# polimi-ispl/deep_prior_interpolation

Hardware: AMD Instinct MI355X
Metric: Adam iters/sec on 3D MultiRes-UNet (whole job over n_gpus; per_gpu beside it); recon SNR(dB) vs ref under config.snr_vs_reference (higher is better)
Workload: dtype f32

## Files before the change

### deep_prior_interpolation_amd/csrc/api.cpp

```cpp
#include <stdarg.h>
#include <string.h>
#include "common.h"

static thread_local char g_err[512] = "";

void dpi_set_error(const char* fmt, ...) {
  va_list ap;
  va_start(ap, fmt);
  vsnprintf(g_err, sizeof(g_err), fmt, ap);
  va_end(ap);
}

int dpi_check_launch(const char* what) {
  const hipError_t e = hipGetLastError();
  if (e != hipSuccess) {
    dpi_set_error("%s: %s", what, hipGetErrorString(e));
    return DPI_E_LAUNCH;
  }
  return DPI_OK;
}

extern "C" const char* dpi_last_error(void) { return g_err; }
extern "C" int dpi_version(void) { return 406; }
extern "C" int dpi_conv_desc_size(void) { return (int)sizeof(dpi_conv_desc); }

extern "C" int dpi_device_info(int device, int* cus, int* lds_bytes, size_t* hbm_bytes, char* name, int name_len) {
  hipDeviceProp_t p;
  const hipError_t e = hipGetDeviceProperties(&p, device);
  if (e != hipSuccess) {
    dpi_set_error("device_info: %s", hipGetErrorString(e));
    return DPI_E_LAUNCH;
  }
  if (cus) *cus = p.multiProcessorCount;
  if (lds_bytes) *lds_bytes = (int)p.sharedMemPerBlock;
  if (hbm_bytes) *hbm_bytes = p.totalGlobalMem;
  if (name && name_len > 0) {
    strncpy(name, p.gcnArchName, name_len - 1);
    name[name_len - 1] = 0;
  }
  return DPI_OK;
}

__global__ void dpi_marker_kernel() {}

extern "C" int dpi_profile_marker(int id, void* stream) {
  DPI_REQUIRE(id >= 1 && id < 65536, "profile_marker: id %d out of range", id);
  dpi_marker_kernel<<<(unsigned)id, 64, 0, (hipStream_t)stream>>>();
  return dpi_check_launch("profile_marker");
}

extern "C" int dpi_set_option(const char* key, int value) {
  DPI_REQUIRE(key != nullptr, "set_option: key is NULL");
  struct Entry { const char* key; int lo, hi; void (*set)(int); };
  static const Entry table[] = {
      {"splitk", 0, 1, dpi_set_splitk},
      {"dual_bwd_data", 0, 1, dpi_set_dual_bwd_data},
      {"bw_pair", 0, 2, dpi_set_bw_pair},
      {"bw_workgroups", 1, 1 << 24, [](int v) { dpi_set_bw_tuning(v, -1); }},
      {"bw_xcd_order", 0, 1, [](int v) { dpi_set_bw_tuning(0, v); }},
      {"mfma_min_cout", 0, 1 << 20, dpi_set_mfma_min_cout},
      {"bwd_weight_mfma_min_cout", 0, 1 << 20, dpi_set_bwd_weight_mfma_min_cout},
      {"fewco_mfma", 0, 1, dpi_set_fewco_mfma},
      {"q4", 0, 2, [](int v) { dpi_set_q4(v, -1); }},
      {"q4_ck", 0, 4, [](int v) { dpi_set_q4(-1, v); }},
      {"q4_debug", 0, 0xFFFF, dpi_set_q4_debug},
      {"bf16_debug", 0, 0x7F, dpi_set_bf16_debug},
  };
  for (const Entry& e : table)
    if (strcmp(key, e.key) == 0) {
      DPI_REQUIRE(value >= e.lo && value <= e.hi && !(strcmp(key, "q4_ck") == 0 && value != 0 && value != 2 && value != 4),
                  "set_option: %s = %d out of range [%d, %d]", key, value, e.lo, e.hi);
      e.set(value);
      return DPI_OK;
    }
  dpi_set_error("set_option: unknown key '%s'", key);
  return DPI_E_ARG;
}
```

### deep_prior_interpolation_amd/csrc/conv_mfma.hip

```cpp
#include "conv_kernels.h"

namespace {

typedef float f32x4 __attribute__((ext_vector_type(4)));

struct MArgs {
  const float* __restrict__ x;
  const float* __restrict__ chain;
  const float* __restrict__ w;
  const float* __restrict__ bias;
  float* __restrict__ y;
  double* __restrict__ partials;
  int Cin, Cout;
  int D, H, W;
  int ntd, nth, ntw;
  long w_out_stride, w_in_stride;
  int accumulate;
  int split_cps;
  const float* __restrict__ x2;
  const float* __restrict__ w2;
  int C2;
  long w2_co_stride, w2_c_stride;
  int xb, yb;
  int ny;
// ... 143 lines not shown
#pragma unroll
      for (int e = 0; e < GV::E; ++e)
        if ((e + 1) * 256 <= GV::NV4 || loff[e] >= 0) {
          float* const p = lds + c * GV::CS + loff[e];
          *reinterpret_cast<f32x2*>(p) = (f32x2){sv[c][e][0], sv[c][e][2]};
          *reinterpret_cast<f32x2*>(p + GV::PW) = (f32x2){sv[c][e][1], sv[c][e][3]};
        }
    return;
  }
#pragma unroll
  for (int c = 0; c < 4; ++c) {
    const Chain t = load_chain(chain, min(c0 + c, Cin - 1));
#pragma unroll
    for (int e = 0; e < GV::E; ++e) {
      const float m = goff[e] >= 0 ? 1.f : 0.f;
      if ((e + 1) * 256 <= GV::NV4 || loff[e] >= 0) {
        float* const p = lds + c * GV::CS + loff[e];
        *reinterpret_cast<f32x2*>(p) = (f32x2){m * apply_chain(t, sv[c][e][0]), m * apply_chain(t, sv[c][e][2])};
        *reinterpret_cast<f32x2*>(p + GV::PW) = (f32x2){m * apply_chain(t, sv[c][e][1]), m * apply_chain(t, sv[c][e][3])};
      }
    }
  }
}

#ifdef DPI_TRACE
__device__ long long g_blk[8192][4];
__device__ long long g_trace[4][64];
#define TR(i) do { if (trc >= 0 && tid == 0) g_trace[trc][i] = clock64(); } while (0)
#define TRC(i) do { if (trc >= 0 && tid == 0 && (i) < 38) g_trace[trc][i] = clock64(); } while (0)
#else
#define TR(i)
#define TRC(i)
#endif
template <int KD, int NR, int NH, bool FLIP, int S = 1, int WPE = 2, bool PERSIST = false, bool TAILPACK = false, bool IOB = false, bool YLOOP = false,
          bool S2V = false>
__global__ __launch_bounds__(256, WPE) void conv_mfma_kernel(MArgs a) {
  static_assert(!YLOOP || (!PERSIST && !TAILPACK), "the channel-tile loop is built for the one-tile-per-workgroup variants without a packed tail");
  static_assert(!S2V || (S == 2 && !FLIP && !PERSIST && !TAILPACK && !IOB && NR < 4), "vectorised stride-2 staging: forward, fp32 tensors, row-split tiles");
  using GV = GeoV2<KD, NR < 4 ? NR : 2, NH>;
  if constexpr (!IOB) { a.xb = 0; a.yb = 0; }
  using G = Geo<KD, NR, NH, S>;
  constexpr int TAPS = KD * 9;
  constexpr int PD = (KD - 1) / 2;
  constexpr int NT = NR * NH;
  __shared__ __attribute__((aligned(16))) float lds[4 * (S2V ? GV::CS : G::CS)];
  __shared__ double red[4][16][2];

  const int tid = threadIdx.x, lane = tid & 63, wid = tid >> 6;
  const int lk = lane >> 4, lj = lane & 15;
  const int ntiles = a.ntd * a.nth * a.ntw;
  int vt0 = blockIdx.x, ytile = blockIdx.y;
  if constexpr (!PERSIST) {
    if (a.ny > 0) {
      const int q8 = ntiles >> 3, r8 = ntiles & 7, xcd = blockIdx.x & 7, j = blockIdx.x >> 3;
      const int i = YLOOP ? j : j / a.ny;
      ytile = YLOOP ? 0 : j - i * a.ny;
      if (i >= q8 + (xcd < r8 ? 1 : 0)) return;
      vt0 = i * 8 + xcd;
    }
  }
  int n0 = ytile * 16;
  const size_t V = (size_t)a.D * a.H * a.W;
  const int Do = (a.D + 2 * PD - KD) / G::SD + 1, Ho = (a.H - 1) / S + 1, Wo = (a.W - 1) / S + 1;
  const size_t Vo = (size_t)Do * Ho * Wo;
#ifdef DPI_TRACE
  const int trc = blockIdx.y != 0 ? -1 : blockIdx.x == 0 ? 0 : blockIdx.x == 1 ? 1 : blockIdx.x == 30 ? 2 : blockIdx.x == 50 ? 3 : -1;
  TR(0);
  if (tid == 0 && blockIdx.y == 0 && blockIdx.x < 8192) {
    g_blk[blockIdx.x][0] = wall_clock64();
    g_blk[blockIdx.x][2] = __builtin_amdgcn_s_getreg(63492);
    g_blk[blockIdx.x][3] = __builtin_amdgcn_s_getreg(63508);
  }
#endif
  auto tile_origin = [&](int vt, int& tile_id, int& od0, int& oh0, int& ow0) {
    tile_id = xcd_tile(vt, ntiles);
    int bt = tile_id;
    const int tw_i = bt % a.ntw; bt /= a.ntw;
    const int th_i = bt % a.nth; bt /= a.nth;
    od0 = bt * G::TZ; oh0 = th_i * G::TY; ow0 = tw_i * G::TW;
  };

  const int wz = G::SLICES ? wid : 0, wh = G::SLICES ? 0 : wid * NR;
  const int lbase = S2V ? lk * GV::CS + wh * 2 * GV::RS + lj : lk * G::CS + wz * G::SD * G::DS + wh * S * G::RS + lj * S;

  int co_w = n0 + lj;
  auto w_ptr = [&](int c0, bool& ok) {
    const int ci = c0 + lk;
    ok = co_w < a.Cout && ci < a.Cin;
    return a.w + (ok ? co_w : 0) * a.w_out_stride + (ok ? ci : 0) * a.w_in_stride;
  };
  auto load_w_raw = [&](float (&wn)[9], int c0, int kd) {
    bool ok;
    const float* __restrict__ wp = w_ptr(c0, ok);
#pragma unroll
    for (int t = 0; t < 9; ++t) wn[t] = wp[FLIP ? (TAPS - 1 - (kd * 9 + t)) : kd * 9 + t];
  };
  auto commit_w = [&](float (&wr)[TAPS], const float (&wn)[9], int c0, int kd) {
    const bool ok = co_w < a.Cout && c0 + lk < a.Cin;
#pragma unroll
    for (int t = 0; t < 9; ++t) wr[kd * 9 + t] = ok ? wn[t] : 0.f;
  };

  const int c_lo = a.split_cps ? (int)blockIdx.z * a.split_cps : 0;
  float* __restrict__ const ybase = a.y + (size_t)blockIdx.z * a.Cout * Vo;
  constexpr int EE = S2V ? GV::E : G::E;
  int goff[EE], loff[EE];
  float wr[TAPS], wn[9], sr[S2V ? 1 : 4][S2V ? 1 : G::E];
  f32x4 sv[S2V ? 4 : 1][S2V ? GV::E : 1];
  auto slots = [&](int od, int oh, int ow) {
    if constexpr (S2V) tile_slots_v<GV>(tid, od * G::SD - PD, oh * 2 - 1, ow * 2 - 4, a.D, a.H, a.W, goff, loff);
    else tile_slots<G>(tid, od * G::SD - PD, oh * S - 1, ow * S - 1, a.D, a.H, a.W, goff, loff);
  };
  auto sload = [&](int c0) {
    if constexpr (S2V) stage_load_v<GV>(sv, a.x, a.Cin, V, c0, goff);
    else stage_load<G>(sr, a.x, a.Cin, V, c0, goff, a.xb);
  };
  auto sstore = [&](int c0) {
    if constexpr (S2V) stage_store_v<GV>(lds, sv, a.chain, a.Cin, c0, goff, loff);
    else stage_store<G>(lds, sr, a.chain, a.Cin, c0, goff, loff, a.xb);
  };
  int vt = vt0, tile_id, od0, oh0, ow0;
  tile_origin(vt, tile_id, od0, oh0, ow0);
  slots(od0, oh0, ow0);
  sload(c_lo);
  {
    bool ok;
    const float* __restrict__ wp = w_ptr(c_lo, ok);
#pragma unroll
    for (int t = 0; t < TAPS; ++t) wr[t] = wp[FLIP ? (TAPS - 1 - t) : t];
#pragma unroll
    for (int t = 0; t < TAPS; ++t) wr[t] = ok ? wr[t] : 0.f;
  }

  constexpr int NTG = (TAPS + 3) / 4;
  const bool tail = TAILPACK && S == 1 && (a.Cin & 3) == 1 && (a.Cin > 4 || a.Cin == 1);
  const int cin_main = a.split_cps ? min(c_lo + a.split_cps, a.Cin) : (tail ? a.Cin - 1 : a.Cin);
  int ttoff[TAILPACK ? NTG : 1];
  float wt[TAILPACK ? NTG : 1];
  if constexpr (TAILPACK) {
#pragma unroll
    for (int g = 0; g < NTG; ++g) {
      const int t = 4 * g + lk;
      const int kd = t / 9, kh = (t / 3) % 3, kw = t % 3;
      ttoff[g] = t < TAPS ? kd * G::DS + kh * G::RS + kw : 0;
      wt[g] = 0.f;
    }
  }
  auto load_tail_w = [&]() {
    if constexpr (TAILPACK) {
      const bool ok = co_w < a.Cout;
      const float* __restrict__ wp = a.w + (ok ? co_w : 0) * a.w_out_stride + (a.Cin - 1) * a.w_in_stride;
#pragma unroll
      for (int g = 0; g < NTG; ++g) {
        const int t = 4 * g + lk < TAPS ? 4 * g + lk : TAPS - 1;
        wt[g] = wp[FLIP ? (TAPS - 1 - t) : t];
      }
    }
  };
  auto commit_tail_w = [&]() {
    if constexpr (TAILPACK) {
#pragma unroll
      for (int g = 0; g < NTG; ++g) wt[g] = (co_w < a.Cout && 4 * g + lk < TAPS) ? wt[g] : 0.f;
    }
  };

  for (;;) {
    const int vt_next = vt + (int)gridDim.x;
    const bool has_next = PERSIST && vt_next < ntiles;
    int tile_n = 0, od_n = 0, oh_n = 0, ow_n = 0;
    if (has_next) tile_origin(vt_next, tile_n, od_n, oh_n, ow_n);

    const int nyt = YLOOP ? a.ny : 1;
    for (int yt = 0; yt < nyt; ++yt) {
    if constexpr (YLOOP) {
      if (yt > 0) {
        n0 = yt * 16; co_w = n0 + lj;
        const bool ok = co_w < a.Cout && c_lo + lk < a.Cin;
#pragma unroll
        for (int t = 0; t < TAPS; ++t) wr[t] = ok ? wr[t] : 0.f;
      }
    }
    f32x4 acc[NT];
#pragma unroll
    for (int t = 0; t < NT; ++t) acc[t] = (f32x4){0.f, 0.f, 0.f, 0.f};
    if (a.accumulate) {
#pragma unroll
      for (int r = 0; r < 4; ++r) {
        const int co = n0 + 4 * lk + r;
#pragma unroll
        for (int t = 0; t < NT; ++t) {
          const int od = od0 + wz, oh = oh0 + wh + t / NH, ow = ow0 + (t % NH) * 16 + lj;
          if (co < a.Cout && od < Do && oh < Ho && ow < Wo) acc[t][r] = dpi_ld(ybase, (size_t)co * Vo + ((size_t)od * Ho + oh) * Wo + ow, a.yb);
        }
      }
    }

    TR(1);
    for (int c0 = c_lo; c0 < cin_main; c0 += 4) {
      if (!YLOOP || yt == 0) {
      __syncthreads();
      TRC(2 + (c0 / 4) * 4);
      sstore(c0);
      TRC(3 + (c0 / 4) * 4);
      __syncthreads();
      TRC(4 + (c0 / 4) * 4);
      }
      const bool more = c0 + 4 < cin_main;
      const bool tail_next = tail && !more;
      if (more || tail_next) sload(c0 + 4);
      else if (has_next) {
        slots(od_n, oh_n, ow_n);
        sload(c_lo);
      }
      float bc[G::NB], bn[G::NB];
      auto load_b = [&](float (&b)[G::NB], int step) {
        const int kd = step / G::NROW, ir = step % G::NROW;
#pragma unroll
        for (int h = 0; h < NH; ++h)
#pragma unroll
          for (int kw = 0; kw < 3; ++kw) {
            if constexpr (S2V)
              b[h * 3 + kw] = lds[lbase + kd * GV::DS + ir * GV::RS + h * 16 + (kw == 1 ? 2 : GV::PW + (kw == 0 ? 1 : 2))];
            else b[h * 3 + kw] = lds[lbase + kd * G::DS + ir * G::RS + h * 16 * S + kw];
          }
      };
      load_b(bc, 0);
      const int cn = more ? c0 + 4 : c_lo;
      if (tail_next) load_tail_w();
#pragma unroll
      for (int step = 0; step < G::NSTEP; ++step) {
        const int kd = step / G::NROW, ir = step % G::NROW;
        if (step + 1 < G::NSTEP) load_b(bn, step + 1);
        if constexpr (!YLOOP) { if (ir == 0) load_w_raw(wn, cn, kd); }
        if (WPE <= 2) __builtin_amdgcn_sched_barrier(0);
#pragma unroll
        for (int kw = 0; kw < 3; ++kw)
#pragma unroll
          for (int kh = 0; kh < 3; ++kh) {
            const int hr = (ir - kh) / S;
            if (ir - kh >= 0 && (ir - kh) % S == 0 && hr < NR) {
#pragma unroll
              for (int h = 0; h < NH; ++h)
                acc[hr * NH + h] = __builtin_amdgcn_mfma_f32_16x16x4f32(wr[(kd * 3 + kh) * 3 + kw], bc[h * 3 + kw], acc[hr * NH + h], 0, 0, 0);
            }
          }
        if (WPE <= 2) __builtin_amdgcn_sched_barrier(0);
#pragma unroll
        for (int i = 0; i < G::NB; ++i) bc[i] = bn[i];
        if constexpr (!YLOOP) { if (ir == G::NROW - 1) commit_w(wr, wn, cn, kd); }
      }
      if (tail_next) commit_tail_w();
      TRC(5 + (c0 / 4) * 4);
    }
    if constexpr (TAILPACK) {
      if (tail && cin_main == 0) { load_tail_w(); commit_tail_w(); }
      if (tail) {
        __syncthreads();
        sstore(cin_main);
        __syncthreads();
        if (has_next) {
          slots(od_n, oh_n, ow_n);
          sload(0);
        }
#pragma unroll
        for (int hr = 0; hr < NR; ++hr) {
          float tb[NH][NTG];
#pragma unroll
          for (int h = 0; h < NH; ++h)
#pragma unroll
            for (int g = 0; g < NTG; ++g) tb[h][g] = lds[lbase + ttoff[g] + hr * G::RS + h * 16];
#pragma unroll
          for (int g = 0; g < NTG; ++g)
#pragma unroll
            for (int h = 0; h < NH; ++h)
              acc[hr * NH + h] = __builtin_amdgcn_mfma_f32_16x16x4f32(wt[g], tb[h][g], acc[hr * NH + h], 0, 0, 0);
        }
      }
    }
    if constexpr (YLOOP) {
      if (yt + 1 < nyt) {
        const int con = (yt + 1) * 16 + lj, ci = c_lo + lk;
        const bool okn = con < a.Cout && ci < a.Cin;
        const float* __restrict__ wp = a.w + (okn ? con : 0) * a.w_out_stride + (okn ? ci : 0) * a.w_in_stride;
#pragma unroll
        for (int t = 0; t < TAPS; ++t) wr[t] = wp[FLIP ? (TAPS - 1 - t) : t];
      }
    }
    if constexpr (FLIP && !PERSIST) if (a.x2 != nullptr) {
      const __amdgpu_buffer_rsrc_t r2 = dpi_buffer_t(a.x2, (size_t)a.C2 * Vo, a.xb);
      int voff[NT];
#pragma unroll
      for (int t = 0; t < NT; ++t) {
        const int od = od0 + wz, oh = oh0 + wh + t / NH, ow = ow0 + (t % NH) * 16 + lj;
        voff[t] = (od < Do && oh < Ho && ow < Wo) ? (od * Ho + oh) * Wo + ow : -1;
      }
      const int nk2 = (a.C2 + 3) >> 2;
      auto load2 = [&](float (&b)[NT], float& wv, int kc) {
        const int c = kc * 4 + lk;
        const bool ok = c < a.C2 && co_w < a.Cout;
        const float wraw = a.w2[(ok ? co_w : 0) * a.w2_co_stride + (ok ? c : 0) * a.w2_c_stride];
        wv = ok ? wraw : 0.f;
        const int cbase = c * (int)Vo;
#pragma unroll
        for (int t = 0; t < NT; ++t)
          b[t] = a.xb ? dpi_buffer_load_bf16(r2, voff[t] >= 0 ? cbase + voff[t] : -1) : dpi_buffer_load(r2, voff[t] >= 0 ? (cbase + voff[t]) * 4 : -4);
      };
      float b0[NT], b1[NT], w0v, w1v;
      load2(b0, w0v, 0);
      for (int kc = 0; kc < nk2; kc += 2) {
        if (kc + 1 < nk2) load2(b1, w1v, kc + 1);
#pragma unroll
        for (int t = 0; t < NT; ++t) acc[t] = __builtin_amdgcn_mfma_f32_16x16x4f32(w0v, b0[t], acc[t], 0, 0, 0);
        if (kc + 1 < nk2) {
          if (kc + 2 < nk2) load2(b0, w0v, kc + 2);
#pragma unroll
          for (int t = 0; t < NT; ++t) acc[t] = __builtin_amdgcn_mfma_f32_16x16x4f32(w1v, b1[t], acc[t], 0, 0, 0);
        }
      }
    }
    TR(40);

    const bool interior = od0 + G::TZ <= Do && oh0 + G::TY <= Ho && ow0 + G::TW <= Wo && n0 + 16 <= a.Cout;
    const int vbase = ((od0 + wz) * Ho + oh0 + wh) * Wo + ow0 + lj;
#pragma unroll
    for (int r = 0; r < 4; ++r) {
      const int co = n0 + 4 * lk + r;
      const bool cok = co < a.Cout;
      const float bv = (a.bias && cok) ? a.bias[co] : 0.f;
      float* __restrict__ yc = dpi_at(ybase, (size_t)(cok ? co : 0) * Vo + vbase, a.yb);
      double s = 0.0, q = 0.0;
      if (a.yb) {
        const bool pairs = !(Wo & 1) && !(Vo & 1) && !((uintptr_t)ybase & 3);
#pragma unroll
        for (int t = 0; t < NT; ++t) {
          const int od = od0 + wz, oh = oh0 + wh + t / NH, ow = ow0 + (t % NH) * 16 + lj;
          const bool ok = interior || (cok && od < Do && oh < Ho && ow < Wo);
          const float v = dpi_round_bf16(acc[t][r] + bv);
          dpi_st_bf16_row(yc, (t / NH) * Wo + (t % NH) * 16, v, ok, pairs, lj);
          if (ok) { s += v; q += (double)v * v; }
        }
      } else if (interior) {
#pragma unroll
        for (int t = 0; t < NT; ++t) {
          const float v = acc[t][r] + bv;
          yc[(t / NH) * Wo + (t % NH) * 16] = v;
          if (a.partials) { s += v; q += (double)v * v; }
        }
      } else {
#pragma unroll
        for (int t = 0; t < NT; ++t) {
          const int od = od0 + wz, oh = oh0 + wh + t / NH, ow = ow0 + (t % NH) * 16 + lj;
          if (cok && od < Do && oh < Ho && ow < Wo) {
            const float v = acc[t][r] + bv;
            yc[(t / NH) * Wo + (t % NH) * 16] = v;
            s += v;
            q += (double)v * v;
          }
        }
      }
      if (a.partials) {
#pragma unroll
        for (int o = 8; o > 0; o >>= 1) { s += __shfl_xor(s, o, 64); q += __shfl_xor(q, o, 64); }
        if (lj == 0) { red[wid][4 * lk + r][0] = s; red[wid][4 * lk + r][1] = q; }
      }
    }
    if (a.partials) {
      __syncthreads();
      if (tid < 32) {
        const int c = tid >> 1, which = tid & 1;
        const double rsum = red[0][c][which] + red[1][c][which] + red[2][c][which] + red[3][c][which];
        if (n0 + c < a.Cout) a.partials[((size_t)tile_id * a.Cout + n0 + c) * 2 + which] = rsum;
      }
    }
    }
    TR(41);
    if (!has_next) break;
    vt = vt_next; tile_id = tile_n; od0 = od_n; oh0 = oh_n; ow0 = ow_n;
  }
#ifdef DPI_TRACE
  if (tid == 0 && blockIdx.y == 0 && blockIdx.x < 8192) g_blk[blockIdx.x][1] = wall_clock64();
#endif
}

struct BwMArgs {
  const float* __restrict__ x;
  const float* __restrict__ chain;
  const float* __restrict__ dy;
  float* __restrict__ ws;
  int Cin, Cout;
  int D, H, W;
  int ntd, nth, ntw, ntiles, tiles_per_chunk;
  int swap;
  int y0;
  int ngroups, nchunks;
  int xb, dyb;
};

template <int KD, int S, int NR, int NH, int NG = 1>
struct BwLds {
  using G = Geo<KD, NR, NH, S>;
  static constexpr int NTQ0 = (4 * KD * 9 + 15) / 16;
  static constexpr int LDSF = NG * (4 * G::CS > 4 * NTQ0 * 256 ? 4 * G::CS : 4 * NTQ0 * 256);
  static constexpr int DYRS = 4 * (4 * NH) + 4;
};

template <int KD, int S, int NR, int NH, int TC, int NG = 1, bool IOB = false>
__device__ __forceinline__ void conv_bwd_weight_mfma_body(const BwMArgs& a_in, float* __restrict__ lds, float* __restrict__ dyl_all, int first_group = -1) {
  BwMArgs a = a_in;
  if constexpr (!IOB) { a.xb = 0; a.dyb = 0; }
  static_assert(NG == 1 || TC == 0, "the column-trimmed tail is a single group");
#ifdef DPI_TRACE
  const int trc = (blockIdx.y == 0 && blockIdx.z == 0 && blockIdx.x < 4) ? (int)blockIdx.x : -1;
  int trn = 0;
#define TRW() do { if (trc >= 0 && threadIdx.x == 0 && trn < 64) g_trace[trc][trn++] = clock64(); } while (0)
// ... 551 lines not shown
  }
}

}

static void dpi_mfma_variant(const dpi_conv_desc* d, int cout, int* nr, int* nh) {
  int Do, Ho, Wo;
  dpi_conv_out_dims(d, &Do, &Ho, &Wo);
  const int tz = d->kd == 3 ? 4 : 1, ty = d->kd == 3 ? 8 : 32;
  const long nb = (long)cdiv(Do, tz) * cdiv(Ho, ty) * cdiv(Wo, 32) * cdiv(cout, 16);
  if (nb >= 512 && d->stride == 1) { *nr = 8; *nh = 2; }
  else { *nr = 2; *nh = Wo > 16 ? 2 : 1; }
}

static bool dpi_mfma_half_tile(const dpi_conv_desc* d, bool flip) {
  const int cin = flip ? d->Cout : d->Cin, cout = flip ? d->Cin : d->Cout;
  int nr, nh;
  dpi_mfma_variant(d, cout, &nr, &nh);
  if (nr != 8 || d->kd != 3) return false;
  if (cin == 1) return true;
  if (cin <= 8) return false;
  return flip || ((cin & 3) == 1);
}

static int dpi_mfma_tiles(const dpi_conv_desc* d, int nr, int nh, int* ntd, int* nth, int* ntw) {
  int Do, Ho, Wo;
  dpi_conv_out_dims(d, &Do, &Ho, &Wo);
  const bool slices = d->kd == 3 && nr >= 4;
  const int tz = slices ? 4 : 1, ty = slices ? nr : 4 * nr;
  *ntd = cdiv(Do, tz); *nth = cdiv(Ho, ty); *ntw = cdiv(Wo, 16 * nh);
  return *ntd * *nth * *ntw;
}

struct MfmaTiling { int nr, nh, ntd, nth, ntw, ntiles; };
static MfmaTiling mfma_tiling(const dpi_conv_desc* d, bool flip) {
  MfmaTiling t{};
  dpi_mfma_variant(d, flip ? d->Cin : d->Cout, &t.nr, &t.nh);
  if (dpi_mfma_half_tile(d, flip)) t.nr = 4;
  t.ntiles = dpi_mfma_tiles(d, t.nr, t.nh, &t.ntd, &t.nth, &t.ntw);
  return t;
}
int dpi_conv_mfma_stat_blocks(const dpi_conv_desc* d, bool flip) { return mfma_tiling(d, flip).ntiles; }

template <int KD, bool FLIP, bool IOB = false>
static void launch_variant(const MArgs& a_in, int nr, int nh, int stride, dim3 grid_in, hipStream_t st) {
  if constexpr (!IOB) {
    if (a_in.xb || a_in.yb) { launch_variant<KD, FLIP, true>(a_in, nr, nh, stride, grid_in, st); return; }
  }
  const bool persistent = stride == 1 && nr == 8 && a_in.Cin > 8;
  MArgs a = a_in;
  dim3 grid = grid_in;
  if (!persistent && grid_in.y > 1) {
    a.ny = (int)grid_in.y;
    grid = dim3(8 * ((grid_in.x + 7) / 8) * grid_in.y, 1, grid_in.z);
  }
  if (stride == 2) {
    if constexpr (!FLIP) {
      if constexpr (!IOB) {
        static const bool s2v = getenv("DPI_NO_S2V") == nullptr;
        if (s2v && a.W % 4 == 0 && (((size_t)a.D * a.H * a.W) & 3) == 0 && ((uintptr_t)a.x & 15) == 0) {
          if (nh == 2) conv_mfma_kernel<KD, 2, 2, false, 2, 2, false, false, false, false, true><<<grid, 256, 0, st>>>(a);
          else conv_mfma_kernel<KD, 2, 1, false, 2, 2, false, false, false, false, true><<<grid, 256, 0, st>>>(a);
          return;
        }
      }
      if (nh == 2) conv_mfma_kernel<KD, 2, 2, false, 2, 2, false, false, IOB><<<grid, 256, 0, st>>>(a);
      else conv_mfma_kernel<KD, 2, 1, false, 2, 2, false, false, IOB><<<grid, 256, 0, st>>>(a);
    }
    return;
  }
  const bool tailpack = (a.Cin & 3) == 1 && (a.Cin > 4 || a.Cin == 1);
  if (nr == 4) {
    if constexpr (KD == 3) {
      if (tailpack) conv_mfma_kernel<KD, 4, 2, FLIP, 1, 3, false, true, IOB><<<grid, 256, 0, st>>>(a);
      else conv_mfma_kernel<KD, 4, 2, FLIP, 1, 3, false, false, IOB><<<grid, 256, 0, st>>>(a);
    }
    return;
  }
  if (nr == 8) {
    static const bool persist = getenv("DPI_NO_PERSIST") == nullptr;
    dim3 pg = grid;
    static const bool yloop = getenv("DPI_YLOOP") != nullptr && getenv("DPI_YLOOP")[0] == '1';
    if constexpr (KD == 3 && FLIP && !IOB) {
      if (yloop && a.Cin <= 4 && a.ny > 1 && a.split_cps == 0 && grid_in.z == 1) {
        conv_mfma_kernel<KD, 8, 2, FLIP, 1, 2, false, false, IOB, true><<<dim3(8 * ((grid_in.x + 7) / 8), 1, 1), 256, 0, st>>>(a);
        return;
      }
    }
    if (a.Cin <= 8) conv_mfma_kernel<KD, 8, 2, FLIP, 1, 3, false, false, IOB><<<grid, 256, 0, st>>>(a);
    else {
      if (persist && grid.x > 512) pg.x = 512;
      if (tailpack) conv_mfma_kernel<KD, 8, 2, FLIP, 1, 2, true, true, IOB><<<pg, 256, 0, st>>>(a);
      else conv_mfma_kernel<KD, 8, 2, FLIP, 1, 2, true, false, IOB><<<pg, 256, 0, st>>>(a);
    }
  }
  else if (nh == 2) conv_mfma_kernel<KD, 2, 2, FLIP, 1, 2, false, false, IOB><<<grid, 256, 0, st>>>(a);
  else conv_mfma_kernel<KD, 2, 1, FLIP, 1, 2, false, false, IOB><<<grid, 256, 0, st>>>(a);
}

#ifdef DPI_TRACE
extern "C" int dpi_debug_read_blocks(long long* out) { return (int)hipMemcpyFromSymbol(out, HIP_SYMBOL(g_blk), sizeof(long long) * 8192 * 4); }
extern "C" int dpi_debug_read_trace(long long* out) { return (int)hipMemcpyFromSymbol(out, HIP_SYMBOL(g_trace), sizeof(long long) * 4 * 64); }
#endif
static int g_splitk = getenv("DPI_SPLITK") ? atoi(getenv("DPI_SPLITK")) : 1;
extern "C" void dpi_set_splitk(int on) { g_splitk = on; }
static int dpi_mfma_splitk(const dpi_conv_desc* d, bool flip) {
  if (!g_splitk || d->k != 3) return 1;
  const int cin = flip ? d->Cout : d->Cin, cout = flip ? d->Cin : d->Cout;
  int nr, nh, a, b, c;
  dpi_mfma_variant(d, cout, &nr, &nh);
  if (nr != 2 || dpi_mfma_half_tile(d, flip)) return 1;
  const long wgs = (long)dpi_mfma_tiles(d, nr, nh, &a, &b, &c) * cdiv(cout, 16);
  const int chunks = cdiv(cin, 4);
  if (wgs > 512 || (wgs > 256 && chunks < 24)) return 1;
  long ns = 1536 / wgs;
  if (ns > chunks / 8) ns = chunks / 8;
  if (ns > 8) ns = 8;
  return ns < 2 ? 1 : (int)ns;
}
size_t dpi_conv_mfma_ws_floats(const dpi_conv_desc* d, bool flip) {
  const int ns = dpi_mfma_splitk(d, flip);
  if (ns < 2) return 0;
  int Do, Ho, Wo;
  dpi_conv_out_dims(d, &Do, &Ho, &Wo);
  return (size_t)ns * (flip ? d->Cin : d->Cout) * Do * Ho * Wo;
}

bool dpi_conv_mfma_second_ok(const dpi_conv_desc* d, bool flip, int C2, bool have_ws) {
  int Do, Ho, Wo;
  dpi_conv_out_dims(d, &Do, &Ho, &Wo);
  if (!flip || d->stride != 1 || C2 < 1 || ((size_t)C2 + 4) * Do * Ho * Wo * sizeof(float) >= ((size_t)1 << 31)) return false;
  int nr, nh;
  dpi_mfma_variant(d, d->Cin, &nr, &nh);
  if (nr == 8 && !dpi_mfma_half_tile(d, flip) && d->Cout > 8) return false;
  return !(have_ws && dpi_mfma_splitk(d, flip) > 1);
}

int dpi_conv_mfma_run(const dpi_conv_desc* d, const float* x, const float* chain, const float* w, const float* bias, float* y,
                      double* partials, bool flip, int accumulate, float* ws, size_t ws_floats, hipStream_t st, const MfmaSecond* sec) {
  const int taps = d->kd * 9;
  const int cin = flip ? d->Cout : d->Cin, cout = flip ? d->Cin : d->Cout;
  const long w_out = flip ? taps : (long)d->Cin * taps, w_in = flip ? (long)d->Cin * taps : taps;
  MArgs a{x, chain, w, bias, y, partials, cin, cout, d->D, d->H, d->W, 0, 0, 0, w_out, w_in, accumulate, 0, nullptr, nullptr, 0, 0, 0,
          dpi_io_in(d, flip), dpi_io_out(d, flip)};
  const MfmaTiling t = mfma_tiling(d, flip);
  const int nr = t.nr, nh = t.nh, ntiles = t.ntiles;
  a.ntd = t.ntd; a.nth = t.nth; a.ntw = t.ntw;
  dim3 grid(ntiles, cdiv(cout, 16));
  if (sec) { a.x2 = sec->x2; a.w2 = sec->w2; a.C2 = sec->C2; a.w2_co_stride = sec->w2_co_stride; a.w2_c_stride = sec->w2_c_stride; }
  const int nsplit = (ws && !sec) ? dpi_mfma_splitk(d, flip) : 1;
  if (nsplit > 1) {
    int Do, Ho, Wo;
    dpi_conv_out_dims(d, &Do, &Ho, &Wo);
    const size_t Vo = (size_t)Do * Ho * Wo;
    DPI_REQUIRE(ws_floats >= (size_t)nsplit * cout * Vo, "conv (split): workspace of %zu floats, need %zu", ws_floats, (size_t)nsplit * cout * Vo);
    a.split_cps = 4 * cdiv(cdiv(cin, 4), nsplit);
    a.y = ws; a.bias = nullptr; a.partials = nullptr; a.accumulate = 0; a.yb = 0;
    grid.z = cdiv(cin, a.split_cps);
    const int nz = (int)grid.z;
    if (d->kd == 3) { if (flip) launch_variant<3, true>(a, nr, nh, d->stride, grid, st); else launch_variant<3, false>(a, nr, nh, d->stride, grid, st); }
    else { if (flip) launch_variant<1, true>(a, nr, nh, d->stride, grid, st); else launch_variant<1, false>(a, nr, nh, d->stride, grid, st); }
    if (int e = dpi_check_launch("conv_mfma (split)")) return e;
    splitk_reduce_kernel<<<dim3(ntiles, cdiv(cout, 4)), 256, 0, st>>>(ws, nz, bias, y, accumulate, partials, cout, Vo, cdivz(Vo, (size_t)ntiles),
                                                                      dpi_io_out(d, flip));
    return dpi_check_launch("splitk_reduce");
  }
  if (d->kd == 3) { if (flip) launch_variant<3, true>(a, nr, nh, d->stride, grid, st); else launch_variant<3, false>(a, nr, nh, d->stride, grid, st); }
  else { if (flip) launch_variant<1, true>(a, nr, nh, d->stride, grid, st); else launch_variant<1, false>(a, nr, nh, d->stride, grid, st); }
  return dpi_check_launch("conv_mfma");
}

static bool mfma_bw_swap_better(const dpi_conv_desc* d) {
  if (d->stride != 1) return false;
  auto util = [](int rows, int staged) { return (double)rows / (16.0 * cdiv(rows, 16)) * staged / (4.0 * cdiv(staged, 4)); };
  return util(d->Cin, d->Cout) > 1.15 * util(d->Cout, d->Cin);
}

static int g_bw_want = getenv("DPI_BW_WANT") ? atoi(getenv("DPI_BW_WANT")) : 2304;
static int g_bw_xcd_order = getenv("DPI_BW_XCD_ORDER") ? atoi(getenv("DPI_BW_XCD_ORDER")) : 0;
extern "C" void dpi_set_bw_tuning(int want_workgroups, int xcd_order) {
  if (want_workgroups > 0) g_bw_want = want_workgroups;
  if (xcd_order >= 0) g_bw_xcd_order = xcd_order;
}
static size_t bw_extra_lds() { static const size_t v = getenv("DPI_BW_EXTRA_LDS") ? (size_t)atoi(getenv("DPI_BW_EXTRA_LDS")) * 1024 : 0; return v; }
struct MfmaBwPlan { int nchunks, tiles_per_chunk, ntiles, ntd, nth, ntw, nr, nh, npairs, nfull, ny; };
static int g_bw_pair = getenv("DPI_BW_PAIR") ? atoi(getenv("DPI_BW_PAIR")) : 2;
extern "C" void dpi_set_bw_pair(int mode) { if (mode >= 0 && mode <= 2) g_bw_pair = mode; }
static MfmaBwPlan mfma_bw_plan(const dpi_conv_desc* d, bool swap = false) {
  MfmaBwPlan p{};
  {
    const int staged = swap ? d->Cout : d->Cin, groups = cdiv(staged, 4);
    const bool s1k3 = d->stride == 1 && d->kd == 3;
    const int tailg = (s1k3 && (staged & 3) == 1) ? 1 : 0;
    p.nfull = groups - tailg;
    p.npairs = (g_bw_pair && s1k3 && !g_bw_xcd_order && p.nfull >= 2 && d->io == 0) ? p.nfull / 2 : 0;
    if (g_bw_pair == 2) {
      int a_, b_, c_;
      if (p.nfull < 4 || dpi_mfma_tiles(d, 8, 2, &a_, &b_, &c_) < 1024) p.npairs = 0;
    }
    p.ny = p.npairs ? p.npairs + (p.nfull & 1) + tailg : groups;
// ... 145 lines not shown
```

### deep_prior_interpolation_amd/csrc/dpi_hip_internal.h

```cpp
#pragma once
#define DPI_INTERNAL __attribute__((visibility("hidden")))
extern "C" {
DPI_INTERNAL void dpi_set_bw_tuning(int want_workgroups, int xcd_order);
DPI_INTERNAL void dpi_set_bf16_debug(int flags);
DPI_INTERNAL void dpi_set_splitk(int on);
DPI_INTERNAL void dpi_set_dual_bwd_data(int on);
DPI_INTERNAL void dpi_set_bw_pair(int mode);
DPI_INTERNAL void dpi_set_mfma_min_cout(int n);
DPI_INTERNAL void dpi_set_bwd_weight_mfma_min_cout(int n);
DPI_INTERNAL void dpi_set_fewco_mfma(int on);
DPI_INTERNAL void dpi_set_q4(int on, int ck);
DPI_INTERNAL void dpi_set_q4_debug(int flags);
}
```

Before: 33.39.

## Compute two output-channel row tiles per workgroup in forward MFMA conv

Adds an RT template parameter so one forward 3x3x3 conv workgroup computes 32 output channels, two 16-row MFMA tiles, reusing each staged input tile from LDS for both. The grid's channel dimension is halved when the pairing applies: fp32 tensors, nr=2/nh=2 tiles, an even number of row tiles, and no split-K. The goal is to halve the input staging and LDS traffic per output channel. In exchange it doubles accumulator and weight registers, which may lower occupancy, and launches fewer workgroups. It is on by default and can be turned off with a conv_row_pair option.

```diff
diff --git a/deep_prior_interpolation_amd/csrc/api.cpp b/deep_prior_interpolation_amd/csrc/api.cpp
--- a/deep_prior_interpolation_amd/csrc/api.cpp
+++ b/deep_prior_interpolation_amd/csrc/api.cpp
@@ -56,6 +56,7 @@
       {"splitk", 0, 1, dpi_set_splitk},
       {"dual_bwd_data", 0, 1, dpi_set_dual_bwd_data},
       {"bw_pair", 0, 2, dpi_set_bw_pair},
+      {"conv_row_pair", 0, 1, dpi_set_conv_row_pair},
       {"bw_workgroups", 1, 1 << 24, [](int v) { dpi_set_bw_tuning(v, -1); }},
       {"bw_xcd_order", 0, 1, [](int v) { dpi_set_bw_tuning(0, v); }},
       {"mfma_min_cout", 0, 1 << 20, dpi_set_mfma_min_cout},
diff --git a/deep_prior_interpolation_amd/csrc/conv_mfma.hip b/deep_prior_interpolation_amd/csrc/conv_mfma.hip
--- a/deep_prior_interpolation_amd/csrc/conv_mfma.hip
+++ b/deep_prior_interpolation_amd/csrc/conv_mfma.hip
@@ -199,34 +199,19 @@
 #define TR(i)
 #define TRC(i)
 #endif
-template <int KD, int NR, int NH, bool FLIP, int S = 1, int WPE = 2, bool PERSIST = false, bool TAILPACK = false, bool IOB = false, bool YLOOP = false,
-          bool S2V = false>
-__global__ __launch_bounds__(256, WPE) void conv_mfma_kernel(MArgs a) {
-  static_assert(!YLOOP || (!PERSIST && !TAILPACK), "the channel-tile loop is built for the one-tile-per-workgroup variants without a packed tail");
-  static_assert(!S2V || (S == 2 && !FLIP && !PERSIST && !TAILPACK && !IOB && NR < 4), "vectorised stride-2 staging: forward, fp32 tensors, row-split tiles");
+template <int KD, int NR, int NH, bool FLIP, int S, int WPE, bool PERSIST, bool TAILPACK, bool IOB, bool YLOOP, bool S2V, int RT>
+__device__ __forceinline__ void conv_mfma_body(const MArgs& a_in, float* __restrict__ lds, double (*__restrict__ red)[4][16][2], int vt0, int n0) {
   using GV = GeoV2<KD, NR < 4 ? NR : 2, NH>;
+  MArgs a = a_in;
   if constexpr (!IOB) { a.xb = 0; a.yb = 0; }
   using G = Geo<KD, NR, NH, S>;
   constexpr int TAPS = KD * 9;
   constexpr int PD = (KD - 1) / 2;
   constexpr int NT = NR * NH;
-  __shared__ __attribute__((aligned(16))) float lds[4 * (S2V ? GV::CS : G::CS)];
-  __shared__ double red[4][16][2];
 
   const int tid = threadIdx.x, lane = tid & 63, wid = tid >> 6;
   const int lk = lane >> 4, lj = lane & 15;
   const int ntiles = a.ntd * a.nth * a.ntw;
-  int vt0 = blockIdx.x, ytile = blockIdx.y;
-  if constexpr (!PERSIST) {
-    if (a.ny > 0) {
-      const int q8 = ntiles >> 3, r8 = ntiles & 7, xcd = blockIdx.x & 7, j = blockIdx.x >> 3;
-      const int i = YLOOP ? j : j / a.ny;
-      ytile = YLOOP ? 0 : j - i * a.ny;
-      if (i >= q8 + (xcd < r8 ? 1 : 0)) return;
-      vt0 = i * 8 + xcd;
-    }
-  }
-  int n0 = ytile * 16;
   const size_t V = (size_t)a.D * a.H * a.W;
   const int Do = (a.D + 2 * PD - KD) / G::SD + 1, Ho = (a.H - 1) / S + 1, Wo = (a.W - 1) / S + 1;
   const size_t Vo = (size_t)Do * Ho * Wo;
@@ -251,28 +236,34 @@
   const int lbase = S2V ? lk * GV::CS + wh * 2 * GV::RS + lj : lk * G::CS + wz * G::SD * G::DS + wh * S * G::RS + lj * S;
 
   int co_w = n0 + lj;
-  auto w_ptr = [&](int c0, bool& ok) {
-    const int ci = c0 + lk;
-    ok = co_w < a.Cout && ci < a.Cin;
-    return a.w + (ok ? co_w : 0) * a.w_out_stride + (ok ? ci : 0) * a.w_in_stride;
+  auto w_ptr = [&](int c0, bool& ok, int rt) {
+    const int ci = c0 + lk, co = co_w + 16 * rt;
+    ok = co < a.Cout && ci < a.Cin;
+    return a.w + (ok ? co : 0) * a.w_out_stride + (ok ? ci : 0) * a.w_in_stride;
   };
-  auto load_w_raw = [&](float (&wn)[9], int c0, int kd) {
-    bool ok;
-    const float* __restrict__ wp = w_ptr(c0, ok);
-#pragma unroll
-    for (int t = 0; t < 9; ++t) wn[t] = wp[FLIP ? (TAPS - 1 - (kd * 9 + t)) : kd * 9 + t];
+  auto load_w_raw = [&](float (&wn)[RT][9], int c0, int kd) {
+#pragma unroll
+    for (int rt = 0; rt < RT; ++rt) {
+      bool ok;
+      const float* __restrict__ wp = w_ptr(c0, ok, rt);
+#pragma unroll
+      for (int t = 0; t < 9; ++t) wn[rt][t] = wp[FLIP ? (TAPS - 1 - (kd * 9 + t)) : kd * 9 + t];
+    }
   };
-  auto commit_w = [&](float (&wr)[TAPS], const float (&wn)[9], int c0, int kd) {
-    const bool ok = co_w < a.Cout && c0 + lk < a.Cin;
-#pragma unroll
-    for (int t = 0; t < 9; ++t) wr[kd * 9 + t] = ok ? wn[t] : 0.f;
+  auto commit_w = [&](float (&wr)[RT][TAPS], const float (&wn)[RT][9], int c0, int kd) {
+#pragma unroll
+    for (int rt = 0; rt < RT; ++rt) {
+      const bool ok = co_w + 16 * rt < a.Cout && c0 + lk < a.Cin;
+#pragma unroll
+      for (int t = 0; t < 9; ++t) wr[rt][kd * 9 + t] = ok ? wn[rt][t] : 0.f;
+    }
   };
 
   const int c_lo = a.split_cps ? (int)blockIdx.z * a.split_cps : 0;
   float* __restrict__ const ybase = a.y + (size_t)blockIdx.z * a.Cout * Vo;
   constexpr int EE = S2V ? GV::E : G::E;
   int goff[EE], loff[EE];
-  float wr[TAPS], wn[9], sr[S2V ? 1 : 4][S2V ? 1 : G::E];
+  float wr[RT][TAPS], wn[RT][9], sr[S2V ? 1 : 4][S2V ? 1 : G::E];
   f32x4 sv[S2V ? 4 : 1][S2V ? GV::E : 1];
   auto slots = [&](int od, int oh, int ow) {
     if constexpr (S2V) tile_slots_v<GV>(tid, od * G::SD - PD, oh * 2 - 1, ow * 2 - 4, a.D, a.H, a.W, goff, loff);
@@ -291,43 +282,54 @@
   slots(od0, oh0, ow0);
   sload(c_lo);
   {
-    bool ok;
-    const float* __restrict__ wp = w_ptr(c_lo, ok);
-#pragma unroll
-    for (int t = 0; t < TAPS; ++t) wr[t] = wp[FLIP ? (TAPS - 1 - t) : t];
-#pragma unroll
-    for (int t = 0; t < TAPS; ++t) wr[t] = ok ? wr[t] : 0.f;
+    bool ok[RT];
+#pragma unroll
+    for (int rt = 0; rt < RT; ++rt) {
+      const float* __restrict__ wp = w_ptr(c_lo, ok[rt], rt);
+#pragma unroll
+      for (int t = 0; t < TAPS; ++t) wr[rt][t] = wp[FLIP ? (TAPS - 1 - t) : t];
+    }
+#pragma unroll
+    for (int rt = 0; rt < RT; ++rt)
+#pragma unroll
+      for (int t = 0; t < TAPS; ++t) wr[rt][t] = ok[rt] ? wr[rt][t] : 0.f;
   }
 
   constexpr int NTG = (TAPS + 3) / 4;
   const bool tail = TAILPACK && S == 1 && (a.Cin & 3) == 1 && (a.Cin > 4 || a.Cin == 1);
   const int cin_main = a.split_cps ? min(c_lo + a.split_cps, a.Cin) : (tail ? a.Cin - 1 : a.Cin);
   int ttoff[TAILPACK ? NTG : 1];
-  float wt[TAILPACK ? NTG : 1];
+  float wt[RT][TAILPACK ? NTG : 1];
   if constexpr (TAILPACK) {
 #pragma unroll
     for (int g = 0; g < NTG; ++g) {
       const int t = 4 * g + lk;
       const int kd = t / 9, kh = (t / 3) % 3, kw = t % 3;
       ttoff[g] = t < TAPS ? kd * G::DS + kh * G::RS + kw : 0;
-      wt[g] = 0.f;
+#pragma unroll
+      for (int rt = 0; rt < RT; ++rt) wt[rt][g] = 0.f;
     }
   }
   auto load_tail_w = [&]() {
     if constexpr (TAILPACK) {
-      const bool ok = co_w < a.Cout;
-      const float* __restrict__ wp = a.w + (ok ? co_w : 0) * a.w_out_stride + (a.Cin - 1) * a.w_in_stride;
-#pragma unroll
-      for (int g = 0; g < NTG; ++g) {
-        const int t = 4 * g + lk < TAPS ? 4 * g + lk : TAPS - 1;
-        wt[g] = wp[FLIP ? (TAPS - 1 - t) : t];
+#pragma unroll
+      for (int rt = 0; rt < RT; ++rt) {
+        const bool ok = co_w + 16 * rt < a.Cout;
+        const float* __restrict__ wp = a.w + (ok ? co_w + 16 * rt : 0) * a.w_out_stride + (a.Cin - 1) * a.w_in_stride;
+#pragma unroll
+        for (int g = 0; g < NTG; ++g) {
+          const int t = 4 * g + lk < TAPS ? 4 * g + lk : TAPS - 1;
+          wt[rt][g] = wp[FLIP ? (TAPS - 1 - t) : t];
+        }
       }
     }
   };
   auto commit_tail_w = [&]() {
     if constexpr (TAILPACK) {
 #pragma unroll
-      for (int g = 0; g < NTG; ++g) wt[g] = (co_w < a.Cout && 4 * g + lk < TAPS) ? wt[g] : 0.f;
+      for (int rt = 0; rt < RT; ++rt)
+#pragma unroll
+        for (int g = 0; g < NTG; ++g) wt[rt][g] = (co_w + 16 * rt < a.Cout && 4 * g + lk < TAPS) ? wt[rt][g] : 0.f;
     }
   };
 
@@ -344,22 +346,26 @@
         n0 = yt * 16; co_w = n0 + lj;
         const bool ok = co_w < a.Cout && c_lo + lk < a.Cin;
 #pragma unroll
-        for (int t = 0; t < TAPS; ++t) wr[t] = ok ? wr[t] : 0.f;
-      }
-    }
-    f32x4 acc[NT];
-#pragma unroll
-    for (int t = 0; t < NT; ++t) acc[t] = (f32x4){0.f, 0.f, 0.f, 0.f};
+        for (int t = 0; t < TAPS; ++t) wr[0][t] = ok ? wr[0][t] : 0.f;
+      }
+    }
+    f32x4 acc[RT][NT];
+#pragma unroll
+    for (int rt = 0; rt < RT; ++rt)
+#pragma unroll
+      for (int t = 0; t < NT; ++t) acc[rt][t] = (f32x4){0.f, 0.f, 0.f, 0.f};
     if (a.accumulate) {
 #pragma unroll
-      for (int r = 0; r < 4; ++r) {
-        const int co = n0 + 4 * lk + r;
-#pragma unroll
-        for (int t = 0; t < NT; ++t) {
-          const int od = od0 + wz, oh = oh0 + wh + t / NH, ow = ow0 + (t % NH) * 16 + lj;
-          if (co < a.Cout && od < Do && oh < Ho && ow < Wo) acc[t][r] = dpi_ld(ybase, (size_t)co * Vo + ((size_t)od * Ho + oh) * Wo + ow, a.yb);
-        }
-      }
+      for (int rt = 0; rt < RT; ++rt)
+#pragma unroll
+        for (int r = 0; r < 4; ++r) {
+          const int co = n0 + 16 * rt + 4 * lk + r;
+#pragma unroll
+          for (int t = 0; t < NT; ++t) {
+            const int od = od0 + wz, oh = oh0 + wh + t / NH, ow = ow0 + (t % NH) * 16 + lj;
+            if (co < a.Cout && od < Do && oh < Ho && ow < Wo) acc[rt][t][r] = dpi_ld(ybase, (size_t)co * Vo + ((size_t)od * Ho + oh) * Wo + ow, a.yb);
+          }
+        }
     }
 
     TR(1);
@@ -408,7 +414,9 @@
             if (ir - kh >= 0 && (ir - kh) % S == 0 && hr < NR) {
 #pragma unroll
               for (int h = 0; h < NH; ++h)
-                acc[hr * NH + h] = __builtin_amdgcn_mfma_f32_16x16x4f32(wr[(kd * 3 + kh) * 3 + kw], bc[h * 3 + kw], acc[hr * NH + h], 0, 0, 0);
+#pragma unroll
+                for (int rt = 0; rt < RT; ++rt)
+                  acc[rt][hr * NH + h] = __builtin_amdgcn_mfma_f32_16x16x4f32(wr[rt][(kd * 3 + kh) * 3 + kw], bc[h * 3 + kw], acc[rt][hr * NH + h], 0, 0, 0);
             }
           }
         if (WPE <= 2) __builtin_amdgcn_sched_barrier(0);
@@ -440,7 +448,9 @@
           for (int g = 0; g < NTG; ++g)
 #pragma unroll
             for (int h = 0; h < NH; ++h)
-              acc[hr * NH + h] = __builtin_amdgcn_mfma_f32_16x16x4f32(wt[g], tb[h][g], acc[hr * NH + h], 0, 0, 0);
+#pragma unroll
+              for (int rt = 0; rt < RT; ++rt)
+                acc[rt][hr * NH + h] = __builtin_amdgcn_mfma_f32_16x16x4f32(wt[rt][g], tb[h][g], acc[rt][hr * NH + h], 0, 0, 0);
         }
       }
     }
@@ -450,7 +460,7 @@
         const bool okn = con < a.Cout && ci < a.Cin;
         const float* __restrict__ wp = a.w + (okn ? con : 0) * a.w_out_stride + (okn ? ci : 0) * a.w_in_stride;
 #pragma unroll
-        for (int t = 0; t < TAPS; ++t) wr[t] = wp[FLIP ? (TAPS - 1 - t) : t];
+        for (int t = 0; t < TAPS; ++t) wr[0][t] = wp[FLIP ? (TAPS - 1 - t) : t];
       }
     }
     if constexpr (FLIP && !PERSIST) if (a.x2 != nullptr) {
@@ -462,36 +472,46 @@
         voff[t] = (od < Do && oh < Ho && ow < Wo) ? (od * Ho + oh) * Wo + ow : -1;
       }
       const int nk2 = (a.C2 + 3) >> 2;
-      auto load2 = [&](float (&b)[NT], float& wv, int kc) {
+      auto load2 = [&](float (&b)[NT], float (&wv)[RT], int kc) {
         const int c = kc * 4 + lk;
-        const bool ok = c < a.C2 && co_w < a.Cout;
-        const float wraw = a.w2[(ok ? co_w : 0) * a.w2_co_stride + (ok ? c : 0) * a.w2_c_stride];
-        wv = ok ? wraw : 0.f;
+#pragma unroll
+        for (int rt = 0; rt < RT; ++rt) {
+          const bool ok = c < a.C2 && co_w + 16 * rt < a.Cout;
+          const float wraw = a.w2[(ok ? co_w + 16 * rt : 0) * a.w2_co_stride + (ok ? c : 0) * a.w2_c_stride];
+          wv[rt] = ok ? wraw : 0.f;
+        }
         const int cbase = c * (int)Vo;
 #pragma unroll
         for (int t = 0; t < NT; ++t)
           b[t] = a.xb ? dpi_buffer_load_bf16(r2, voff[t] >= 0 ? cbase + voff[t] : -1) : dpi_buffer_load(r2, voff[t] >= 0 ? (cbase + voff[t]) * 4 : -4);
       };
-      float b0[NT], b1[NT], w0v, w1v;
+      float b0[NT], b1[NT], w0v[RT], w1v[RT];
       load2(b0, w0v, 0);
       for (int kc = 0; kc < nk2; kc += 2) {
         if (kc + 1 < nk2) load2(b1, w1v, kc + 1);
 #pragma unroll
-        for (int t = 0; t < NT; ++t) acc[t] = __builtin_amdgcn_mfma_f32_16x16x4f32(w0v, b0[t], acc[t], 0, 0, 0);
+        for (int t = 0; t < NT; ++t)
+#pragma unroll
+          for (int rt = 0; rt < RT; ++rt) acc[rt][t] = __builtin_amdgcn_mfma_f32_16x16x4f32(w0v[rt], b0[t], acc[rt][t], 0, 0, 0);
         if (kc + 1 < nk2) {
           if (kc + 2 < nk2) load2(b0, w0v, kc + 2);
 #pragma unroll
-          for (int t = 0; t < NT; ++t) acc[t] = __builtin_amdgcn_mfma_f32_16x16x4f32(w1v, b1[t], acc[t], 0, 0, 0);
+          for (int t = 0; t < NT; ++t)
+#pragma unroll
+            for (int rt = 0; rt < RT; ++rt) acc[rt][t] = __builtin_amdgcn_mfma_f32_16x16x4f32(w1v[rt], b1[t], acc[rt][t], 0, 0, 0);
         }
       }
     }
     TR(40);
 
-    const bool interior = od0 + G::TZ <= Do && oh0 + G::TY <= Ho && ow0 + G::TW <= Wo && n0 + 16 <= a.Cout;
     const int vbase = ((od0 + wz) * Ho + oh0 + wh) * Wo + ow0 + lj;
 #pragma unroll
+    for (int rt = 0; rt < RT; ++rt) {
+    const int n0r = n0 + 16 * rt;
+    const bool interior = od0 + G::TZ <= Do && oh0 + G::TY <= Ho && ow0 + G::TW <= Wo && n0r + 16 <= a.Cout;
+#pragma unroll
     for (int r = 0; r < 4; ++r) {
-      const int co = n0 + 4 * lk + r;
+      const int co = n0r + 4 * lk + r;
       const bool cok = co < a.Cout;
       const float bv = (a.bias && cok) ? a.bias[co] : 0.f;
       float* __restrict__ yc = dpi_at(ybase, (size_t)(cok ? co : 0) * Vo + vbase, a.yb);
@@ -502,14 +522,14 @@
         for (int t = 0; t < NT; ++t) {
           const int od = od0 + wz, oh = oh0 + wh + t / NH, ow = ow0 + (t % NH) * 16 + lj;
           const bool ok = interior || (cok && od < Do && oh < Ho && ow < Wo);
-          const float v = dpi_round_bf16(acc[t][r] + bv);
+          const float v = dpi_round_bf16(acc[rt][t][r] + bv);
           dpi_st_bf16_row(yc, (t / NH) * Wo + (t % NH) * 16, v, ok, pairs, lj);
           if (ok) { s += v; q += (double)v * v; }
         }
       } else if (interior) {
 #pragma unroll
         for (int t = 0; t < NT; ++t) {
-          const float v = acc[t][r] + bv;
+          const float v = acc[rt][t][r] + bv;
           yc[(t / NH) * Wo + (t % NH) * 16] = v;
           if (a.partials) { s += v; q += (double)v * v; }
         }
@@ -518,7 +538,7 @@
         for (int t = 0; t < NT; ++t) {
           const int od = od0 + wz, oh = oh0 + wh + t / NH, ow = ow0 + (t % NH) * 16 + lj;
           if (cok && od < Do && oh < Ho && ow < Wo) {
-            const float v = acc[t][r] + bv;
+            const float v = acc[rt][t][r] + bv;
             yc[(t / NH) * Wo + (t % NH) * 16] = v;
             s += v;
             q += (double)v * v;
@@ -528,15 +548,16 @@
       if (a.partials) {
 #pragma unroll
         for (int o = 8; o > 0; o >>= 1) { s += __shfl_xor(s, o, 64); q += __shfl_xor(q, o, 64); }
-        if (lj == 0) { red[wid][4 * lk + r][0] = s; red[wid][4 * lk + r][1] = q; }
-      }
+        if (lj == 0) { red[rt][wid][4 * lk + r][0] = s; red[rt][wid][4 * lk + r][1] = q; }
+      }
+    }
     }
     if (a.partials) {
       __syncthreads();
-      if (tid < 32) {
-        const int c = tid >> 1, which = tid & 1;
-        const double rsum = red[0][c][which] + red[1][c][which] + red[2][c][which] + red[3][c][which];
-        if (n0 + c < a.Cout) a.partials[((size_t)tile_id * a.Cout + n0 + c) * 2 + which] = rsum;
+      if (tid < 32 * RT) {
+        const int rt = tid >> 5, c = (tid & 31) >> 1, which = tid & 1;
+        const double rsum = red[rt][0][c][which] + red[rt][1][c][which] + red[rt][2][c][which] + red[rt][3][c][which];
+        if (n0 + 16 * rt + c < a.Cout) a.partials[((size_t)tile_id * a.Cout + n0 + 16 * rt + c) * 2 + which] = rsum;
       }
     }
     }
@@ -547,6 +568,30 @@
 #ifdef DPI_TRACE
   if (tid == 0 && blockIdx.y == 0 && blockIdx.x < 8192) g_blk[blockIdx.x][1] = wall_clock64();
 #endif
+}
+
+template <int KD, int NR, int NH, bool FLIP, int S = 1, int WPE = 2, bool PERSIST = false, bool TAILPACK = false, bool IOB = false, bool YLOOP = false,
+          bool S2V = false, int RT = 1>
+__global__ __launch_bounds__(256, WPE) void conv_mfma_kernel(MArgs a) {
+  static_assert(!YLOOP || (!PERSIST && !TAILPACK), "the channel-tile loop is built for the one-tile-per-workgroup variants without a packed tail");
+  static_assert(!S2V || (S == 2 && !FLIP && !PERSIST && !TAILPACK && !IOB && NR < 4), "vectorised stride-2 staging: forward, fp32 tensors, row-split tiles");
+  static_assert(RT == 1 || (RT == 2 && !YLOOP && !IOB), "row pairs: fp32 tensors, one spatial tile at a time");
+  using GV = GeoV2<KD, NR < 4 ? NR : 2, NH>;
+  using G = Geo<KD, NR, NH, S>;
+  __shared__ __attribute__((aligned(16))) float lds[4 * (S2V ? GV::CS : G::CS)];
+  __shared__ double red[RT][4][16][2];
+  int vt0 = blockIdx.x, col = blockIdx.y;
+  if constexpr (!PERSIST) {
+    if (a.ny > 0) {
+      const int ntiles = a.ntd * a.nth * a.ntw;
+      const int q8 = ntiles >> 3, r8 = ntiles & 7, xcd = blockIdx.x & 7, j = blockIdx.x >> 3;
+      const int i = YLOOP ? j : j / a.ny;
+      col = YLOOP ? 0 : j - i * a.ny;
+      if (i >= q8 + (xcd < r8 ? 1 : 0)) return;
+      vt0 = i * 8 + xcd;
+    }
+  }
+  conv_mfma_body<KD, NR, NH, FLIP, S, WPE, PERSIST, TAILPACK, IOB, YLOOP, S2V, RT>(a, lds, red, vt0, col * 16 * RT);
 }
 
 struct BwMArgs {
@@ -1164,18 +1209,25 @@
   return *ntd * *nth * *ntw;
 }
 
-struct MfmaTiling { int nr, nh, ntd, nth, ntw, ntiles; };
+static int g_row_pair = 1;
+extern "C" void dpi_set_conv_row_pair(int on) { g_row_pair = on; }
+
+struct MfmaTiling { int nr, nh, ntd, nth, ntw, ntiles, rt; };
 static MfmaTiling mfma_tiling(const dpi_conv_desc* d, bool flip) {
   MfmaTiling t{};
   dpi_mfma_variant(d, flip ? d->Cin : d->Cout, &t.nr, &t.nh);
   if (dpi_mfma_half_tile(d, flip)) t.nr = 4;
+  const int rows = cdiv(d->Cout, 16);
+  const bool pair = g_row_pair && !flip && d->kd == 3 && d->Cin > 4 && !dpi_io_in(d, flip) && !dpi_io_out(d, flip) && t.nr == 2 && t.nh == 2 &&
+                    (rows & 1) == 0 && rows >= (d->stride == 2 ? 2 : 4);
+  t.rt = pair ? 2 : 1;
   t.ntiles = dpi_mfma_tiles(d, t.nr, t.nh, &t.ntd, &t.nth, &t.ntw);
   return t;
 }
 int dpi_conv_mfma_stat_blocks(const dpi_conv_desc* d, bool flip) { return mfma_tiling(d, flip).ntiles; }
 
 template <int KD, bool FLIP, bool IOB = false>
-static void launch_variant(const MArgs& a_in, int nr, int nh, int stride, dim3 grid_in, hipStream_t st) {
+static void launch_variant(const MArgs& a_in, int nr, int nh, int stride, dim3 grid_in, hipStream_t st, int rt = 1) {
   if constexpr (!IOB) {
     if (a_in.xb || a_in.yb) { launch_variant<KD, FLIP, true>(a_in, nr, nh, stride, grid_in, st); return; }
   }
@@ -1191,10 +1243,16 @@
       if constexpr (!IOB) {
         static const bool s2v = getenv("DPI_NO_S2V") == nullptr;
         if (s2v && a.W % 4 == 0 && (((size_t)a.D * a.H * a.W) & 3) == 0 && ((uintptr_t)a.x & 15) == 0) {
+          if constexpr (KD == 3) {
+            if (rt == 2) { conv_mfma_kernel<KD, 2, 2, false, 2, 2, false, false, false, false, true, 2><<<grid, 256, 0, st>>>(a); return; }
+          }
           if (nh == 2) conv_mfma_kernel<KD, 2, 2, false, 2, 2, false, false, false, false, true><<<grid, 256, 0, st>>>(a);
           else conv_mfma_kernel<KD, 2, 1, false, 2, 2, false, false, false, false, true><<<grid, 256, 0, st>>>(a);
           return;
         }
+      }
+      if constexpr (KD == 3 && !IOB) {
+        if (rt == 2) { conv_mfma_kernel<KD, 2, 2, false, 2, 2, false, false, false, false, false, 2><<<grid, 256, 0, st>>>(a); return; }
       }
       if (nh == 2) conv_mfma_kernel<KD, 2, 2, false, 2, 2, false, false, IOB><<<grid, 256, 0, st>>>(a);
       else conv_mfma_kernel<KD, 2, 1, false, 2, 2, false, false, IOB><<<grid, 256, 0, st>>>(a);
@@ -1226,8 +1284,13 @@
       else conv_mfma_kernel<KD, 8, 2, FLIP, 1, 2, true, false, IOB><<<pg, 256, 0, st>>>(a);
     }
   }
-  else if (nh == 2) conv_mfma_kernel<KD, 2, 2, FLIP, 1, 2, false, false, IOB><<<grid, 256, 0, st>>>(a);
-  else conv_mfma_kernel<KD, 2, 1, FLIP, 1, 2, false, false, IOB><<<grid, 256, 0, st>>>(a);
+  else {
+    if constexpr (KD == 3 && !FLIP && !IOB) {
+      if (rt == 2) { conv_mfma_kernel<KD, 2, 2, false, 1, 2, false, false, false, false, false, 2><<<grid, 256, 0, st>>>(a); return; }
+    }
+    if (nh == 2) conv_mfma_kernel<KD, 2, 2, FLIP, 1, 2, false, false, IOB><<<grid, 256, 0, st>>>(a);
+    else conv_mfma_kernel<KD, 2, 1, FLIP, 1, 2, false, false, IOB><<<grid, 256, 0, st>>>(a);
+  }
 }
 
 #ifdef DPI_TRACE
@@ -1278,9 +1341,10 @@
   const MfmaTiling t = mfma_tiling(d, flip);
   const int nr = t.nr, nh = t.nh, ntiles = t.ntiles;
   a.ntd = t.ntd; a.nth = t.nth; a.ntw = t.ntw;
-  dim3 grid(ntiles, cdiv(cout, 16));
   if (sec) { a.x2 = sec->x2; a.w2 = sec->w2; a.C2 = sec->C2; a.w2_co_stride = sec->w2_co_stride; a.w2_c_stride = sec->w2_c_stride; }
   const int nsplit = (ws && !sec) ? dpi_mfma_splitk(d, flip) : 1;
+  const int rt = nsplit > 1 ? 1 : t.rt;
+  dim3 grid(ntiles, cdiv(cdiv(cout, 16), rt));
   if (nsplit > 1) {
     int Do, Ho, Wo;
     dpi_conv_out_dims(d, &Do, &Ho, &Wo);
@@ -1297,7 +1361,7 @@
                                                                       dpi_io_out(d, flip));
     return dpi_check_launch("splitk_reduce");
   }
-  if (d->kd == 3) { if (flip) launch_variant<3, true>(a, nr, nh, d->stride, grid, st); else launch_variant<3, false>(a, nr, nh, d->stride, grid, st); }
+  if (d->kd == 3) { if (flip) launch_variant<3, true>(a, nr, nh, d->stride, grid, st, rt); else launch_variant<3, false>(a, nr, nh, d->stride, grid, st, rt); }
   else { if (flip) launch_variant<1, true>(a, nr, nh, d->stride, grid, st); else launch_variant<1, false>(a, nr, nh, d->stride, grid, st); }
   return dpi_check_launch("conv_mfma");
 }
diff --git a/deep_prior_interpolation_amd/csrc/dpi_hip_internal.h b/deep_prior_interpolation_amd/csrc/dpi_hip_internal.h
--- a/deep_prior_interpolation_amd/csrc/dpi_hip_internal.h
+++ b/deep_prior_interpolation_amd/csrc/dpi_hip_internal.h
@@ -6,6 +6,7 @@
 DPI_INTERNAL void dpi_set_splitk(int on);
 DPI_INTERNAL void dpi_set_dual_bwd_data(int on);
 DPI_INTERNAL void dpi_set_bw_pair(int mode);
+DPI_INTERNAL void dpi_set_conv_row_pair(int on);
 DPI_INTERNAL void dpi_set_mfma_min_cout(int n);
 DPI_INTERNAL void dpi_set_bwd_weight_mfma_min_cout(int n);
 DPI_INTERNAL void dpi_set_fewco_mfma(int on);
```

After: 33.48, median of 2. Within noise of the previous version (+0.3%).
